# JasonQSY/Articulation3D

Hardware: AMD Instinct MI355X
Metric: frames/sec through PlaneRCNN detector at 480x640 (higher is better)
Workload: dtype f32 storage and accumulation; operands enter the matrix pipe with a 22-bit significand under ONE power-of-two block exponent per image (per ROI behind the poolers, per layer for filters): x*s = h + l in fp16, three fp16 MFMAs per k step (h.h + h.l + l.h). Elementwise law |y - y64| <= c (2^-22 sum|x|; 1 GPU; BASELINE configs[2]: full PlaneRCNN detector (ResNet50-FPN + RPN + ROIAlign + box/mask/plane/axis heads + depth head + NMS + mask paste + plane-offset LSQ + record pack), random-init weights with calibrated BN, synthetic 480x640 uint8 frames resident in HBM (arithmetic: see `dtype`)

## Files before the change

articulation3d_amd/csrc/conv_gemm.hip:

```cpp
#include "conv_common.h"
#include <stdarg.h>
#include <stdio.h>

static int conv_check(const a3d_conv_desc *d) {
    if (!d || (!d->x && !d->x_h2) || !d->w || (!d->y && !d->dot_y)) return A3D_ERR_ARG;
    if ((d->dot_w || d->dot_y) && d->phase != 5) return A3D_ERR_ARG;
    if (d->x_h2 && d->precision != 3) return A3D_ERR_ARG;
    if (d->B <= 0 || d->Ho <= 0 || d->Wo <= 0 || d->Cout <= 0) return A3D_ERR_ARG;
    if ((d->Cout & 3) || (d->Kpad & 31) || d->splitk < 1) return A3D_ERR_ARG;
    if (d->stem) {
        if (d->KH != 7 || d->KW != 7 || d->stride != 2 || d->pad != 3 || d->Kpad != 224 || d->Cin2 || d->ups) return A3D_ERR_ARG;
    } else {
        if ((d->Cin & 31) || (d->Cin2 & 31) || (d->Cin2 && !d->x2 && !d->x2_h2)) return A3D_ERR_ARG;
        if (d->Kpad < d->KH * d->KW * (d->Cin + d->Cin2)) return A3D_ERR_ARG;
    }
    if (d->pixshuf && (d->Cout & 15)) return A3D_ERR_ARG;
    if (d->phase < 0 || d->phase > 5 || (d->phase == 5 && d->precision != 3 && d->precision != 2)) return A3D_ERR_ARG;
    if (d->gate && (d->pixshuf || d->phase)) return A3D_ERR_ARG;
    if (d->io_bf16 && d->precision != 1) return A3D_ERR_ARG;
    if (d->splitk > 1 && !d->workspace) return A3D_ERR_ARG;
    if ((size_t)d->B * d->H * d->W >= ((size_t)1 << 31)) return A3D_ERR_UNSUPPORTED;
    return A3D_OK;
}

static thread_local char g_last_variant[160] = "";
void a3d_note_variant(const char *fmt, ...) {
    va_list ap;
    va_start(ap, fmt);
    vsnprintf(g_last_variant, sizeof(g_last_variant), fmt, ap);
    va_end(ap);
}
extern "C" const char *a3d_last_conv_variant(void) { return g_last_variant; }

extern "C" size_t a3d_conv_workspace_bytes(const a3d_conv_desc *d) {
    if (!d) return 0;
    if (d->tune == 0 && a3d_wino_fused_eligible(d)) return 0;
    if ((d->tune == 0 || d->tune == 7 || d->tune == 8 || (d->tune >= 23 && d->tune <= 25) || d->tune >= 200) && a3d_wino_eligible(d)) return a3d_wino_workspace_bytes(d);
    if (d->splitk <= 1) return 0;
    return (size_t)d->splitk * d->B * d->Ho * d->Wo * d->Cout * sizeof(float);
}

extern "C" int a3d_conv2d_nhwc_f32(const a3d_conv_desc *d, void *stream) {
    const int rc = conv_check(d);
    if (rc != A3D_OK) return rc;
    hipStream_t s = (hipStream_t)stream;
    a3d_begin();
    if (d->precision == 1) return a3d_conv_launch_bf16(d, s);
    if (d->precision == 2) {
        if ((d->tune == 0 || d->tune == 8 || d->tune == 24 || d->tune == 25) && d->workspace && d->w_wino && d->w_wino_x3 && ((d->Cin + d->Cin2) & 31) == 0 && a3d_wino_eligible(d)) return a3d_conv_launch_wino(d, s);
        return a3d_conv_launch_bf16x3(d, s);
    }
    if (d->precision == 3 && d->x_h2) return a3d_conv_launch_bf16x3_wide(d, s);
    if (d->precision == 3) {
        if ((d->tune == 0 || d->tune == 23 || d->tune == 24) && d->workspace && d->w_wino && d->w_wino_x3 && ((d->Cin + d->Cin2) & 31) == 0 && a3d_wino_eligible(d))
            return a3d_conv_launch_wino(d, s);
        return a3d_conv_launch_bf16x3(d, s);
    }
    if (d->precision != 0) return A3D_ERR_ARG;
    if (d->tune == 0 && a3d_wino_fused_eligible(d)) return a3d_conv_launch_wino_fused(d, s);
    if ((d->tune == 0 || d->tune == 7 || d->tune >= 200) && d->workspace && a3d_wino_eligible(d)) return a3d_conv_launch_wino(d, s);
    if (d->tune == 0 || d->tune == 6) {
        const int r1 = a3d_conv_launch_pw(d, s, d->tune == 6);
        if (r1 != A3D_ERR_UNSUPPORTED) return r1;
    }
    if (d->tune == 1) return A3D_ERR_UNSUPPORTED;
    return a3d_conv_launch_v2(d, s);
}

extern "C" int a3d_version(void) { return 1; }
```

articulation3d_amd/csrc/conv_wino.hip:

```cpp
#include "conv_common.h"
#include <stdlib.h>

typedef unsigned int u32x4 __attribute__((ext_vector_type(4)));

__global__ __launch_bounds__(256) void wino_input_kernel(const float *__restrict__ x, const float *__restrict__ x2,
                                                         float *__restrict__ V, int B, int H, int W, int Cin, int Cin2,
                                                         int ups, int Ty, int Tx) {
    const int C = Cin + Cin2, C4 = C >> 2;
    const int Hl = ups ? 2 * H : H, Wl = ups ? 2 * W : W;
    const size_t T = (size_t)B * Ty * Tx;
    const size_t total = T * C4;
    for (size_t i = (size_t)blockIdx.x * blockDim.x + threadIdx.x; i < total; i += (size_t)gridDim.x * blockDim.x) {
        const int c = (int)(i % C4) * 4;
        const size_t t = i / C4;
        const int tx = (int)(t % Tx);
        const size_t r = t / Tx;
        const int ty = (int)(r % Ty);
        const int b = (int)(r / Ty);
        const bool second = c >= Cin;
        const float *src = second ? x2 : x;
        const int cs = second ? Cin2 : Cin, cc = second ? c - Cin : c;
        f32x4 d[4][4];
#pragma unroll
        for (int p = 0; p < 4; ++p) {
            const int ly = 2 * ty - 1 + p;
#pragma unroll
            for (int q = 0; q < 4; ++q) {
                const int lx = 2 * tx - 1 + q;
                f32x4 v = {0.f, 0.f, 0.f, 0.f};
                if ((unsigned)ly < (unsigned)Hl && (unsigned)lx < (unsigned)Wl) {
                    const int sy = ups ? ly >> 1 : ly, sx = ups ? lx >> 1 : lx;
                    v = *reinterpret_cast<const f32x4 *>(src + (((size_t)b * H + sy) * W + sx) * cs + cc);
                }
                d[p][q] = v;
            }
        }
        f32x4 m[4][4];
#pragma unroll
        for (int q = 0; q < 4; ++q) {
            m[0][q] = d[0][q] - d[2][q];
            m[1][q] = d[1][q] + d[2][q];
            m[2][q] = d[2][q] - d[1][q];
            m[3][q] = d[1][q] - d[3][q];
        }
#pragma unroll
        for (int u = 0; u < 4; ++u) {
            const f32x4 v0 = m[u][0] - m[u][2], v1 = m[u][1] + m[u][2], v2 = m[u][2] - m[u][1], v3 = m[u][1] - m[u][3];
            float *o = V + ((size_t)(u * 4) * T + t) * C + c;
            *reinterpret_cast<f32x4 *>(o) = v0;
            *reinterpret_cast<f32x4 *>(o + T * C) = v1;
            *reinterpret_cast<f32x4 *>(o + 2 * T * C) = v2;
            *reinterpret_cast<f32x4 *>(o + 3 * T * C) = v3;
        }
    }
}

typedef unsigned int wi_u32x2 __attribute__((ext_vector_type(2)));
typedef unsigned int wi_u32x4 __attribute__((ext_vector_type(4)));
__global__ __launch_bounds__(256) void wino_input_h2_kernel(const float *__restrict__ x, const float *__restrict__ x2, unsigned char *__restrict__ Vs,
                                                            const float *__restrict__ in_amax, const float *__restrict__ in_amax2, int B, int H, int W,
                                                            int Cin, int Cin2, int ups, int Ty, int Tx, int t_off, int t_total) {
    const int C = Cin + Cin2;
    const int Hl = ups ? 2 * H : H, Wl = ups ? 2 * W : W;
    const size_t T = (size_t)B * Ty * Tx;
    const size_t tile = (size_t)t_total * 64;
    const int KC = C >> 5;
    const size_t witems = ((T + 7) / 8) * KC;
    const int lane = threadIdx.x & 63;
    for (size_t w = (size_t)blockIdx.x * (blockDim.x >> 6) + (threadIdx.x >> 6); w < witems; w += (size_t)gridDim.x * (blockDim.x >> 6)) {
        const int kcw = (int)(w % KC);
        const size_t t = (w / KC) * 8 + (lane >> 3);
        if (t >= T) continue;
        const int c = kcw * 32 + (lane & 7) * 4;
        const int tx = (int)(t % Tx);
        const size_t r = t / Tx;
        const int ty = (int)(r % Ty);
        const int b = (int)(r / Ty);
        const bool second = c >= Cin;
        const float *src = second ? x2 : x;
        const int cs = second ? Cin2 : Cin, cc = second ? c - Cin : c;
        float am = in_amax[b];
        if (in_amax2) am = fmaxf(am, in_amax2[b]);
        const float sv = 0.25f * a3d_pow2_scale(am);
        f32x4 d[4][4];
#pragma unroll
        for (int p = 0; p < 4; ++p) {
            const int ly = 2 * ty - 1 + p;
#pragma unroll
            for (int q = 0; q < 4; ++q) {
                const int lx = 2 * tx - 1 + q;
                f32x4 v = {0.f, 0.f, 0.f, 0.f};
                if ((unsigned)ly < (unsigned)Hl && (unsigned)lx < (unsigned)Wl) {
                    const int sy = ups ? ly >> 1 : ly, sx = ups ? lx >> 1 : lx;
                    v = *reinterpret_cast<const f32x4 *>(src + (((size_t)b * H + sy) * W + sx) * cs + cc);
                }
                d[p][q] = v;
            }
        }
        f32x4 m[4][4];
#pragma unroll
        for (int q = 0; q < 4; ++q) {
            m[0][q] = d[0][q] - d[2][q];
            m[1][q] = d[1][q] + d[2][q];
            m[2][q] = d[2][q] - d[1][q];
            m[3][q] = d[1][q] - d[3][q];
        }
        const int kc = c >> 5;
        unsigned char *oh = Vs + (size_t)kc * 2 * tile + ((size_t)t_off + t) * 64 + (c & 31) * 2;
        const size_t pstride = (size_t)KC * 2 * tile;
#pragma unroll
        for (int u = 0; u < 4; ++u) {
            const f32x4 vv[4] = {m[u][0] - m[u][2], m[u][1] + m[u][2], m[u][2] - m[u][1], m[u][1] - m[u][3]};
#pragma unroll
            for (int v = 0; v < 4; ++v) {
                h16x4 h, l;
                a3d_split2h(vv[v], sv, h, l);
                *reinterpret_cast<h16x4 *>(oh) = h;
                *reinterpret_cast<h16x4 *>(oh + tile) = l;
                oh += pstride;
            }
        }
    }
}

struct WinoArgs {
    const float *V;
    const float *U;
    const float *scale, *shift;
    const float *gate;
    float *y;
    int T, C, Cout, B, Hl, Wl, Ty, Tx, act;
    const __bf16 *U3;
    float *y_amax;
    const float *in_amax, *in_amax2;
    float w_scale;
    float *M;
    int abl;
    int Toff, Ttot;
    struct Levels {
        int n;
        int t0[6];
        int Ty[5], Tx[5], Hl[5], Wl[5];
        float *y[5];
        const float *in_amax[5];
        float *y_amax[5];
    } lv;
};
__device__ __forceinline__ void wino_level_of(const WinoArgs::Levels &L, const int t, int &l, int &tl) {
    l = 0;
#pragma unroll
    for (int k = 1; k < 5; ++k) l = (k < L.n && t >= L.t0[k]) ? k : l;
    int base = L.t0[0];
#pragma unroll
    for (int k = 1; k < 5; ++k) base = l == k ? L.t0[k] : base;
    tl = t - base;
}
template <typename V>
__device__ __forceinline__ V wino_level_sel(const V (&arr)[5], const int l) {
    V v = arr[0];
#pragma unroll
    for (int k = 1; k < 5; ++k) v = l == k ? arr[k] : v;
    return v;
}

__device__ __forceinline__ float wino_v_scale(const WinoArgs &a, const int b) {
    float m = a.in_amax[b];
    if (a.in_amax2) m = fmaxf(m, a.in_amax2[b]);
    return 0.25f * a3d_pow2_scale(m);
}

template <int TN, int BKT>
__global__ __launch_bounds__(256, TN == 1 ? 3 : 1) void wino_gemm_kernel(const WinoArgs a, const int ntiles, const int nblk) {
    constexpr int BM = 64, BN = 2 * TN * 32;
    constexpr int LK = BKT + 4, TPR = BKT / 4, RPP = 256 / TPR;
    constexpr int XR = (BM + RPP - 1) / RPP, WR = BN / RPP;
    constexpr int BUF = (BM + BN) * LK;
    static_assert(BN % RPP == 0 && (BM % RPP == 0 || BM < RPP), "loader pass must tile the operand rows");
    __shared__ __attribute__((aligned(16))) float lds[2 * BUF];
    __shared__ __attribute__((aligned(16))) float ss[2 * BN];

    const int tid = threadIdx.x, lane = tid & 63, wave = tid >> 6;
    const int wm = wave >> 1, wn = wave & 1;
    const int logical = a3d_xcd_remap(blockIdx.x, nblk);
    const int mt = logical / ntiles, nt = logical - mt * ntiles;
    const int t0 = mt * BM, n0 = nt * BN;
    const int lr = tid / TPR, lc = (tid % TPR) * 4;
    const size_t vplane = (size_t)a.T * a.C, uplane = (size_t)a.Cout * a.C;
    const unsigned vbytes = (unsigned)(vplane * 4), ubytes = (unsigned)(uplane * 4);
    const int KC = a.C / BKT;
    const int NIT = 16 * KC;

    int xoff[XR], woff[WR];
#pragma unroll
    for (int i = 0; i < XR; ++i) {
        const int rrow = lr + RPP * i;
        const int t = t0 + rrow;
        xoff[i] = (rrow < BM && t < a.T) ? (t * a.C + lc) * 4 : -1;
    }
#pragma unroll
    for (int i = 0; i < WR; ++i) {
        const int n = n0 + lr + RPP * i;
        woff[i] = n < a.Cout ? (n * a.C + lc) * 4 : -1;
    }
    f32x4 xsA[XR], wsA[WR], xsB[XR], wsB[WR];
// ... 1052 lines not shown
    *reinterpret_cast<bf16x4 *>(d + (size_t)rows * chunk) = m;
    *reinterpret_cast<bf16x4 *>(d + (size_t)rows * chunk * 2) = l;
}

extern "C" int a3d_split_bf16x3_chunk(const float *src, void *dst, int outer, int rows, int cols, int chunk, void *stream) {
    if (!src || !dst || outer <= 0 || rows <= 0 || cols <= 0 || (chunk != 16 && chunk != 32) || cols % chunk) return A3D_ERR_ARG;
    a3d_begin();
    const size_t total = (size_t)outer * rows * cols;
    hipLaunchKernelGGL(split_bf16x3_kernel, dim3((unsigned)((total / 4 + 255) / 256)), dim3(256), 0, (hipStream_t)stream, src, (__bf16 *)dst, rows, cols, chunk,
                       total);
    return a3d_check_launch();
}

__global__ __launch_bounds__(256) void split_f16x2_kernel(const float *__restrict__ src, _Float16 *__restrict__ dst, int rows, int cols, int chunk, float scale,
                                                          size_t total) {
    const size_t i = ((size_t)blockIdx.x * 256 + threadIdx.x) * 4;
    if (i >= total) return;
    const size_t per = (size_t)rows * cols;
    const size_t o = i / per, r = i - o * per;
    const int n = (int)(r / cols), c = (int)(r - (size_t)n * cols);
    h16x4 h, l;
    a3d_split2h(*reinterpret_cast<const f32x4 *>(src + i), scale, h, l);
    _Float16 *d = dst + o * 2 * per + ((size_t)(c / chunk) * 2 * rows + n) * chunk + (c % chunk);
    *reinterpret_cast<h16x4 *>(d) = h;
    *reinterpret_cast<h16x4 *>(d + (size_t)rows * chunk) = l;
}

extern "C" int a3d_split_f16x2_chunk(const float *src, void *dst, int outer, int rows, int cols, int chunk, float scale, void *stream) {
    if (!src || !dst || outer <= 0 || rows <= 0 || cols <= 0 || (chunk != 16 && chunk != 32) || cols % chunk || !(scale > 0.f)) return A3D_ERR_ARG;
    a3d_begin();
    const size_t total = (size_t)outer * rows * cols;
    hipLaunchKernelGGL(split_f16x2_kernel, dim3((unsigned)((total / 4 + 255) / 256)), dim3(256), 0, (hipStream_t)stream, src, (_Float16 *)dst, rows, cols, chunk,
                       scale, total);
    return a3d_check_launch();
}

extern "C" int a3d_split_bf16x3(const float *src, void *dst, int outer, int rows, int cols, void *stream) {
    return a3d_split_bf16x3_chunk(src, dst, outer, rows, cols, 32, stream);
}

int a3d_wino_eligible(const a3d_conv_desc *d) {
    if (!d->w_wino) return 0;
    if (d->KH != 3 || d->KW != 3 || d->stride != 1 || d->pad != 1) return 0;
    if (d->res || d->pixshuf || d->stem || d->splitk != 1 || d->m_dev) return 0;
    if (((d->Cin + d->Cin2) & 15) || (d->Cin & 3) || (d->Cin2 & 3) || (d->Cout & 3)) return 0;
    const int Hl = d->ups ? 2 * d->H : d->H, Wl = d->ups ? 2 * d->W : d->W;
    const size_t T = (size_t)d->B * ((Hl + 1) / 2) * ((Wl + 1) / 2);
    const size_t C = (size_t)d->Cin + d->Cin2;
    if (T * C * 4 >= ((size_t)1 << 32) || (size_t)d->Cout * C * 4 >= ((size_t)1 << 32)) return 0;
    return 1;
}

size_t a3d_wino_workspace_bytes(const a3d_conv_desc *d) {
    const int Hl = d->ups ? 2 * d->H : d->H, Wl = d->ups ? 2 * d->W : d->W;
    size_t T = (size_t)d->B * ((Hl + 1) / 2) * ((Wl + 1) / 2);
    if (d->precision == 3 && d->wino_t_total > 0) T = (size_t)d->wino_t_total;
    return 16 * T * ((size_t)d->Cin + d->Cin2) * sizeof(float);
}

extern "C" size_t a3d_wino_m_bytes(const a3d_conv_desc *d) {
    const long ps_max = a3d_dev_knob("A3D_WINO_PS_BLOCKS", 48);
    if (!d || d->precision != 3 || !a3d_wino_eligible(d)) return 0;
    const int C = d->Cin + d->Cin2;
    if ((C & 63) || ((d->Cout + 63) / 64) % 2 != 0) return 0;
    const int Hl = d->ups ? 2 * d->H : d->H, Wl = d->ups ? 2 * d->W : d->W;
    const size_t T = (size_t)d->B * ((Hl + 1) / 2) * ((Wl + 1) / 2);
    const long blocks4 = (long)((T + 127) / 128) * ((d->Cout + X3W_BN - 1) / X3W_BN);
    if (blocks4 > ps_max) return 0;
    return 16 * T * (size_t)d->Cout * sizeof(float);
}

static int wino_launch_input(const a3d_conv_desc *d, hipStream_t s) {
    const int Hl = d->ups ? 2 * d->H : d->H, Wl = d->ups ? 2 * d->W : d->W;
    const int Ty = (Hl + 1) / 2, Tx = (Wl + 1) / 2;
    const int C = d->Cin + d->Cin2;
    const size_t T = (size_t)d->B * Ty * Tx;
    const size_t total = T * (C / 4);
    size_t blocks = (total + 255) / 256;
    if (blocks > 16384) blocks = 16384;
    if (d->precision == 3) {
        if ((C & 31) || !d->in_amax) return A3D_ERR_ARG;
        if (d->wino_t_total && (d->wino_t_off < 0 || (size_t)d->wino_t_off + T > (size_t)d->wino_t_total)) return A3D_ERR_ARG;
        if ((size_t)(d->wino_t_total ? d->wino_t_total : T) * C * 4 >= ((size_t)1 << 32)) return A3D_ERR_UNSUPPORTED;
        hipLaunchKernelGGL(wino_input_h2_kernel, dim3((int)blocks), dim3(256), 0, s, d->x, d->x2, reinterpret_cast<unsigned char *>(d->workspace), d->in_amax,
                           d->in_amax2, d->B, d->H, d->W, d->Cin, d->Cin2, d->ups, Ty, Tx, d->wino_t_total ? d->wino_t_off : 0, d->wino_t_total ? d->wino_t_total : (int)T);
        return A3D_OK;
    }
    hipLaunchKernelGGL(wino_input_kernel, dim3((int)blocks), dim3(256), 0, s, d->x, d->x2, d->workspace, d->B, d->H, d->W,
                       d->Cin, d->Cin2, d->ups, Ty, Tx);
    return A3D_OK;
}

static int wino_launch_gemm(const a3d_conv_desc *d, hipStream_t s) {
    const int Hl = d->ups ? 2 * d->H : d->H, Wl = d->ups ? 2 * d->W : d->W;
    const int Ty = (Hl + 1) / 2, Tx = (Wl + 1) / 2;
    const size_t T = (size_t)d->B * Ty * Tx;
    WinoArgs a;
    a.V = d->workspace;
    a.U = d->w_wino;
    a.scale = d->scale;
    a.shift = d->shift;
    a.gate = d->gate;
    a.y = d->y;
    a.T = (int)T;
    a.C = d->Cin + d->Cin2;
    a.Cout = d->Cout;
    a.B = d->B;
    a.Hl = Hl;
    a.Wl = Wl;
    a.Ty = Ty;
    a.Tx = Tx;
    a.act = d->act;
    const int mtiles = (int)((T + 63) / 64);
    a.U3 = nullptr;
    a.y_amax = d->y_amax;
    a.in_amax = d->in_amax;
    a.in_amax2 = d->in_amax2;
    a.w_scale = d->w_scale;
    a.M = nullptr;
    a.abl = (int)a3d_dev_knob("A3D_WINO_ABL", 0);
    a.Toff = 0;
    a.Ttot = (int)T;
    a.lv.n = 1;
    for (int k = 0; k < 5; ++k) {
        a.lv.t0[k] = k == 0 ? 0 : (int)T;
        a.lv.Ty[k] = Ty;
        a.lv.Tx[k] = Tx;
        a.lv.Hl[k] = Hl;
        a.lv.Wl[k] = Wl;
        a.lv.y[k] = d->y;
        a.lv.in_amax[k] = d->in_amax;
        a.lv.y_amax[k] = d->y_amax;
    }
    a.lv.t0[5] = (int)T;
    if (d->wino_t_total) {
        if (d->precision != 3 || d->wino_t_off < 0 || (size_t)d->wino_t_off + T > (size_t)d->wino_t_total) return A3D_ERR_ARG;
        a.Toff = d->wino_t_off;
        a.Ttot = d->wino_t_total;
    }
    if (d->precision == 3) {
        if (!d->w_wino_x3 || (a.C & 31) || !d->in_amax || !(d->w_scale > 0.f) || ((d->Cout + 63) / 64) % 2 != 0 ||
            (size_t)16 * d->Cout * a.C * 4 >= ((size_t)1 << 32))
            return A3D_ERR_ARG;
        a.U3 = reinterpret_cast<const __bf16 *>(d->w_wino_x3);
        const int nt = (d->Cout + X3W_BN - 1) / X3W_BN;
        const int wmx = d->tune == 24 ? 2 : 4;
        static a3d_attr_once attr3;
        if (attr3.needed()) {
            if (hipFuncSetAttribute((const void *)wino_gemm_x3w_kernel<2, true>, hipFuncAttributeMaxDynamicSharedMemorySize, x3w_lds_bytes(2, 2)) != hipSuccess ||
                hipFuncSetAttribute((const void *)wino_gemm_x3w_kernel<4, true>, hipFuncAttributeMaxDynamicSharedMemorySize, x3w_lds_bytes(4, 2)) != hipSuccess ||
                hipFuncSetAttribute((const void *)wino_gemm_x3w_kernel<4, true, false, 1>, hipFuncAttributeMaxDynamicSharedMemorySize, x3w_lds_bytes(4, 2)) != hipSuccess ||
                hipFuncSetAttribute((const void *)wino_gemm_x3w_kernel<2, true, true>, hipFuncAttributeMaxDynamicSharedMemorySize, x3w_lds_bytes(2, 2)) != hipSuccess)
                return A3D_ERR_LAUNCH;
            attr3.mark();
        }
        if (d->wino_m && a3d_wino_m_bytes(d)) {
            a.M = d->wino_m;
            a3d_note_variant("wino_gemm_h2w_kernel<2> planes + wino_fold_kernel");
            hipLaunchKernelGGL((wino_gemm_x3w_kernel<2, true, true>), dim3(mtiles * nt, 16), dim3(256), x3w_lds_bytes(2, 2), s, a, nt, mtiles * nt);
            const size_t threads = T * (size_t)(d->Cout / 4);
            hipLaunchKernelGGL(wino_fold_kernel, dim3((unsigned)((threads + 255) / 256)), dim3(256), 0, s, a);
            return A3D_OK;
        }
        a3d_note_variant("wino_gemm_h2w_kernel<%d>", wmx);
        if (wmx == 4) {
            const int m4 = (int)((T + 127) / 128);
            if (d->tune == 23) hipLaunchKernelGGL((wino_gemm_x3w_kernel<4, true>), dim3(m4 * nt), dim3(512), x3w_lds_bytes(4, 2), s, a, nt, m4 * nt);
            else hipLaunchKernelGGL((wino_gemm_x3w_kernel<4, true, false, 1>), dim3(m4 * nt), dim3(512), x3w_lds_bytes(4, 2), s, a, nt, m4 * nt);
// ... 142 lines not shown
```

articulation3d_amd/ops.py:

```python
from __future__ import annotations

import ctypes as C
import math
import os
from dataclasses import dataclass
from typing import List, Optional, Sequence, Tuple

import torch

from . import _lib
from ._lib import ACT_LEAKY, ACT_NONE, ACT_RELU

GROUP_CAP = 1024
fptr_t = C.c_void_p

CONV_TIMING: Optional[list] = None

DEFAULT_PRECISION = int(os.environ.get("A3D_PRECISION", "3"))


def last_conv_variant() -> str:
    return _lib.lib().a3d_last_conv_variant().decode()


# ... 285 lines not shown
    publish()
    return t.data_ptr()


def _conv_desc(p: PackedConv, B: int, H: int, W: int, Cin: int, Cin2: int, Ho: int, Wo: int, act: Optional[int] = None,
               res_ups: bool = False) -> "_lib.ConvDesc":
    d = _lib.ConvDesc()
    d.w, d.scale, d.shift = _p(p.w), _p(p.scale), _p(p.shift)
    d.B, d.H, d.W, d.Cin, d.Cin2 = B, H, W, Cin, Cin2
    d.Ho, d.Wo, d.Cout = Ho, Wo, p.cols
    d.KH, d.KW, d.stride, d.pad = p.KH, p.KW, p.stride, p.pad
    d.Kpad, d.act = p.Kpad, p.act if act is None else act
    d.res_ups, d.pixshuf, d.stem, d.phase, d.splitk = int(res_ups), int(p.pixshuf), int(p.stem), int(p.phase), 1
    return d


def _y_amax(out: torch.Tensor) -> int:
    ya = getattr(out, "_a3d_amax", None)
    if ya is None or ya.numel() != out.shape[0]:
        ya = out._a3d_amax = amax_slot(out.shape[0], out.device)
    return ya.data_ptr()


def _image_blocks(B: int, nb: int, *ts):
    for s in range(0, B, nb):
        e = min(s + nb, B)
        yield s, e, [t if t is None or e - s == B else keep_amax(t[s:e], _amax_rows(t, s, e)) for t in ts]


CONV_TIMING_ONLY: Optional[frozenset] = None
_TIMED_VARIANTS: dict = {}
_ERR_UNSUPPORTED = -3


def _launch(fn, *args, precision: Optional[int] = None, rec=None, unsupported: bool = False) -> bool:
    global _LAST_PRECISION
    if precision is not None:
        _LAST_PRECISION = precision
    timed = CONV_TIMING is not None and rec is not None
    if timed:
        label, fl, shape, ex, pipe, key = rec()
        if CONV_TIMING_ONLY is not None:
            known = label if label is not None else _TIMED_VARIANTS.get(key)
            timed = known is None or known in CONV_TIMING_ONLY
        if timed:
            e0, e1 = (torch.cuda.Event(enable_timing=True) for _ in range(2))
            e0.record()
    rc = fn(*args, _stream())
    if rc:
        if unsupported and rc == _ERR_UNSUPPORTED:
            return False
        _lib.check(rc, fn.__name__)
    if timed:
        e1.record()
        if label is None:
            label = _TIMED_VARIANTS[key] = last_conv_variant()
        CONV_TIMING.append((label, fl, e0, e1, shape, ex, pipe, _stream()))
    return True


_WINO_SHARE: Optional[dict] = None
WINO_SHARE_ENABLED = os.environ.get("A3D_WINO_SHARE", "1") != "0"


class share_wino_input:

    def __init__(self, tensors: Sequence[torch.Tensor]):
        self.map = {t.data_ptr(): [t, None] for t in tensors} if WINO_SHARE_ENABLED else {}

    def __enter__(self):
        global _WINO_SHARE
        self.prev, _WINO_SHARE = _WINO_SHARE, self.map
        return self

    def __exit__(self, *exc):
        global _WINO_SHARE
        _WINO_SHARE = self.prev
        self.map = {}
        return False


_ADDR_LIMIT = (1 << 32) - 1
WINO_LEVELS = os.environ.get("A3D_WINO_LEVELS", "1") != "0"


def conv2d_levels(xs: Sequence[torch.Tensor], p: PackedConv) -> list:
    xs = list(xs)
    ok = (WINO_LEVELS and DEFAULT_PRECISION == 3 and AUDIT is None and 2 <= len(xs) <= 5 and p.w_wino is not None
          and p.pin_precision != 2 and p.KH == 3 and p.stride == 1 and p.pad == 1 and not (p.stem or p.phase or p.pixshuf)
          and all(x.is_cuda and x.dtype == torch.float32 and x.shape[0] == xs[0].shape[0] and x.shape[3] == p.Cin for x in xs)
          and p.Cin % 32 == 0 and p.Cin >= 256 and -(-p.cols // 64) % 2 == 0)
    if ok and _WINO_SHARE is not None:
        ok = all((_WINO_SHARE.get(x.data_ptr()) or [None, None])[1] is None for x in xs)
    tiles = [x.shape[0] * ((x.shape[1] + 1) // 2) * ((x.shape[2] + 1) // 2) for x in xs]
    total = sum(tiles)
    if not ok or total * p.Cin * 4 > _ADDR_LIMIT:
        return [conv2d(x, p) for x in xs]
    dev = xs[0].device
    w_h2, u_scale = weight_planes(p, "w_wino_h2"), filter_scale(p, wino=True)
    ws = torch.empty(16 * total * p.Cin, device=dev, dtype=torch.float32)
    descs = (_lib.ConvDesc * len(xs))()
    outs, off = [], 0
    shape = lambda: f"{xs[0].shape[0]}x[{'+'.join(str(x.shape[1]) + 'x' + str(x.shape[2]) for x in xs)}]x{p.Cin}->{p.cols} k3 s1"
    for k, x in enumerate(xs):
        _req(x)
        B, H, W, Cin = x.shape
        out = torch.empty((B, H, W, p.cols), device=dev, dtype=torch.float32)
        descs[k] = _conv_desc(p, B, H, W, Cin, 0, H, W)
        d = descs[k]
        d.x, d.y, d.precision = _p(x), _p(out), 3
        d.w_wino, d.w_wino_x3, d.w_scale = p.w_wino.data_ptr(), w_h2, u_scale
        d.in_amax = amax_of(x).data_ptr()
        d.y_amax = _y_amax(out)
        d.workspace = ws.data_ptr()
        d.wino_t_off, d.wino_t_total = off, total
        _launch(_lib.lib().a3d_wino_input_transform, C.byref(d), precision=3, rec=lambda: ("wino_input_kernel", 0.0, shape(), 0.0, "none", None))
        if _WINO_SHARE is not None:
            ent = _WINO_SHARE.get(x.data_ptr())
            if ent is not None and ent[0].shape == x.shape:
                ent[1:] = [ws, 3, (off, total)]
        off += tiles[k]
        outs.append(out)

    def rec():
        px = sum(x.shape[0] * x.shape[1] * x.shape[2] for x in xs)
        return "wino_gemm_h2w_kernel<4>", 2.0 * px * p.cols * 9 * p.Cin, shape(), 2.0 * total * 16 * p.cols * p.Cin, "f16x3", None

    _launch(_lib.lib().a3d_wino_gemm_levels, descs, len(xs), precision=3, rec=rec)
    return outs


def conv2d(x: torch.Tensor, p: PackedConv, *, x2: Optional[torch.Tensor] = None, res: Optional[torch.Tensor] = None,
           res_ups: bool = False, ups: bool = False, act: Optional[int] = None, splitk: int = 1,
           m_dev: Optional[torch.Tensor] = None, out: Optional[torch.Tensor] = None, tune: int = 0,
           wino: Optional[bool] = None, gate: Optional[torch.Tensor] = None, precision=None, out_dtype=None, dot=None) -> torch.Tensor:
    if AUDIT is not None and not AUDIT.busy and precision is None and x.dtype == torch.float32 and out_dtype is None and not p.phase:
        return AUDIT.conv2d(x, p, x2=x2, res=res, res_ups=res_ups, ups=ups, act=act, splitk=splitk, m_dev=m_dev, out=out, tune=tune, wino=wino, gate=gate)
    if x.dtype == torch.float16:
        if splitk != 1 or m_dev is not None or gate is not None or tune or out_dtype is not None or ups or dot is not None or wino or precision not in (None, 3):
            raise RuntimeError("pre-split (float16) activations run the dual-DMA fp16x2 kernel only: splitk, m_dev, gate, tune, out_dtype, ups, dot, "
                               "wino and any precision other than 3 are not available with them")
        return _conv2d_presplit(x, p, x2=x2, res=res, res_ups=res_ups, act=act, out=out)
    if out_dtype is not None or x.dtype == torch.bfloat16 or (res is not None and res.dtype == torch.bfloat16) or (gate is not None and gate.dtype == torch.bfloat16):
        return _conv2d_bf16_storage(x, p, res=res, res_ups=res_ups, act=act, out=out, gate=gate, precision=precision, out_dtype=out_dtype, tune=tune)
    _req(x)
    B = x.shape[0]
    if B > 1:
        Hl_, Wl_ = (2 * x.shape[1], 2 * x.shape[2]) if ups else (x.shape[1], x.shape[2])
        Ho_ = x.shape[1] if p.phase else (Hl_ + 2 * p.pad - p.KH) // p.stride + 1
        Wo_ = x.shape[2] if p.phase else (Wl_ + 2 * p.pad - p.KW) // p.stride + 1
        per_in = x.shape[1] * x.shape[2] * max(x.shape[3], 0 if x2 is None else x2.shape[3]) * 4
        per_out = Ho_ * Wo_ * p.cols * 4 * (4 if 0 < p.phase < 5 else 1) * max(1, int(splitk))
        if dot is not None:
            per_out = 9 * 4 * Ho_ * Wo_ * 4
        per_v = ((Hl_ + 1) // 2) * ((Wl_ + 1) // 2) * (x.shape[3] + (0 if x2 is None else x2.shape[3])) * 4 if p.w_wino is not None else 0
        per = max(per_in, per_out, per_v, 1)
        if B * per > _ADDR_LIMIT:
            if dot is not None:
                raise RuntimeError("tap-product epilogue (dot): the batch must fit one launch")
            return _conv2d_blocks(x, p, max(1, _ADDR_LIMIT // per), (Ho_, Wo_), x2=x2, res=res, res_ups=res_ups, ups=ups, act=act, splitk=splitk,
                                  m_dev=m_dev, out=out, tune=tune, wino=wino, gate=gate, precision=precision)
    return _conv2d_launch(x, p, x2=x2, res=res, res_ups=res_ups, ups=ups, act=act, splitk=splitk, m_dev=m_dev, out=out, tune=tune,
                          wino=wino, gate=gate, precision=precision, dot=dot)


def _conv2d_blocks(x, p, nb, hw_out, *, x2, res, out, gate, m_dev, **kw):
    B = x.shape[0]
    Ho, Wo = hw_out
    if out is None:
        shape = (B, 2 * Ho, 2 * Wo, p.cols // 4) if p.pixshuf else (B, Ho, Wo, p.cols)
        out = torch.empty(shape, device=x.device, dtype=torch.float32)
    recorded = []
    for s, e, (xb, x2b, rb, gb) in _image_blocks(B, nb, x, x2, res, gate):
        md = None if m_dev is None else (m_dev.reshape(1) - s).clamp(0, e - s).to(torch.int32)
        o = out[s:e]
        ya = getattr(out, "_a3d_amax", None)
        if ya is not None and ya.numel() == B:
            o._a3d_amax = ya[s:e]
        _conv2d_launch(xb, p, x2=x2b, res=rb, out=o, gate=gb, m_dev=md, **kw)
        recorded.append(getattr(o, "_a3d_amax", None))
    if getattr(out, "_a3d_amax", None) is None and all(r is not None for r in recorded):
        out._a3d_amax = torch.cat(recorded)
    return out


BF16_SPLITK = os.environ.get("A3D_BF16_SPLITK", "1") != "0"
BF16_SPLITK_AUTO = False
_BF16_SK_CFG = tuple(int(v) for v in os.environ.get("A3D_BF16_SPLITK_CFG", "128,256,12,24,8").split(","))


def _bf16_splitk(M: int, cols: int, Kpad: int) -> int:
    tiles = -(-M // 128) * -(-cols // 64)
    nk = Kpad // 32
    maxtiles, target, per, minnk, cap = _BF16_SK_CFG
    if not BF16_SPLITK or tiles > maxtiles or nk < minnk:
        return 1
    return int(max(1, min(cap, nk // per, target // tiles)))

# ... 48 lines not shown
    def rec():
        fl = 2.0 * B * Ho * Wo * p.cols * p.KH * p.KW * p.Cin
        return None, fl, f"{B}x{H}x{W}x{Cin}->{p.cols} k{p.KH} s{p.stride} io{int(d.io_bf16)}", fl, "bf16", key

    _launch(_lib.lib().a3d_conv2d_nhwc_f32, C.byref(d), precision=1, rec=rec)
    return out


def presplit_f16x2(x: torch.Tensor, x2: Optional[torch.Tensor] = None):
    _req(x)
    B, n = x.shape[0], x.numel() // x.shape[0]
    ax, ax2 = amax_of(x), (None if x2 is None else amax_of(_req(x2)))
    outs = []
    for t in ((x,) if x2 is None else (x, x2)):
        nt = t.numel() // B
        o = torch.empty(tuple(t.shape[:-1]) + (t.shape[-1] // 16, 2, 16), device=t.device, dtype=torch.float16)
        _lib.check(_lib.lib().a3d_presplit_f16x2(t.data_ptr(), o.data_ptr(), ax.data_ptr(), _p(ax2), B, nt, _stream()), "a3d_presplit_f16x2")
        o._a3d_amax = ax if x2 is None else torch.maximum(ax, ax2)
        outs.append(o)
    return outs[0] if x2 is None else tuple(outs)


def _conv2d_presplit(x, p: PackedConv, *, x2=None, res=None, res_ups=False, act=None, out=None) -> torch.Tensor:
    if DEFAULT_PRECISION != 3:
        raise RuntimeError("pre-split activations belong to the fp16x2 arithmetic (A3D_PRECISION=3)")
    ok = lambda t: t.is_cuda and t.is_contiguous() and t.dtype == torch.float16 and t.dim() == 6 and t.shape[4:] == (2, 16)
    if not ok(x) or (x2 is not None and not ok(x2)):
        raise RuntimeError("expected contiguous pre-split fp16 tensors [B, H, W, C/16, 2, 16]")
    B, H, W = x.shape[:3]
    Cin = x.shape[3] * 16
    Cin2 = 0 if x2 is None else x2.shape[3] * 16
    assert Cin + Cin2 == p.Cin and not (p.stem or p.pixshuf or p.phase) and p.presplit and p.Kpad == p.KH * p.KW * p.Cin, "plain direct layers only"
    Ho = (H + 2 * p.pad - p.KH) // p.stride + 1
    Wo = (W + 2 * p.pad - p.KW) // p.stride + 1
    if out is None:
        out = torch.empty((B, Ho, Wo, p.cols), device=x.device, dtype=torch.float32)
    per_image = max(H * W * max(Cin, Cin2), Ho * Wo * p.cols) * 4
    if B * per_image > _ADDR_LIMIT:
        ya = out._a3d_amax = amax_slot(B, x.device)
        for s, e, (xb, x2b, rb) in _image_blocks(B, max(1, _ADDR_LIMIT // per_image), x, x2, res):
            o = out[s:e]
            o._a3d_amax = ya[s:e]
            _conv2d_presplit(xb, p, x2=x2b, res=rb, res_ups=res_ups, act=act, out=o)
        return out
    a = getattr(x, "_a3d_amax", None)
    if a is None or a.numel() != B:
        raise RuntimeError("a pre-split tensor carries the per-image maxima it was scaled by (_a3d_amax)")
    d = _conv_desc(p, B, H, W, Cin, Cin2, Ho, Wo, act=act, res_ups=res_ups)
    d.x_h2, d.x2_h2, d.res, d.y = x.data_ptr(), _p(x2), _p(res), out.data_ptr()
    d.precision = 3
    d.tune = int(os.environ.get("A3D_XD_TUNE", "0"))
    d.in_amax = a.data_ptr()
    d.w_scale, d.w_x3 = filter_scale(p), weight_planes(p, "w_h2")
    d.y_amax = _y_amax(out)

    def rec():
        fl = 2.0 * B * Ho * Wo * p.cols * p.KH * p.KW * p.Cin
        return None, fl, f"{B}x{H}x{W}x{Cin + Cin2}->{p.cols} k{p.KH} s{p.stride} presplit", fl, "f16x3", (id(p), B, H, W, Cin, Cin2, "presplit")

    _launch(_lib.lib().a3d_conv2d_nhwc_f32, C.byref(d), precision=3, rec=rec)
    return out


class _amax_rows:

    def __init__(self, t, s, e):
        a = getattr(t, "_a3d_amax", None)
        self._a3d_amax = None if a is None or a.numel() != t.shape[0] else a[s:e]
        self.shape = (e - s,)


def _check_res(res: torch.Tensor, B: int, Ho: int, Wo: int, cols: int, res_ups: bool) -> None:
    _req(res)
    want = (B, Ho >> 1, Wo >> 1, cols) if res_ups else (B, Ho, Wo, cols)
    if tuple(res.shape) != want or (res_ups and (Ho % 2 or Wo % 2)):
        raise ValueError(f"residual of shape {tuple(res.shape)} for an output grid [{B}, {Ho}, {Wo}, {cols}]{' (res_ups)' if res_ups else ''}: expected {want}")


_PIPE = {0: "f32", 1: "bf16", 2: "bf16x6", 3: "f16x3"}


def _arithmetic(p: PackedConv, default: int, wino_tune: int, precision, Cin: int, Cin2: int, *, ups: bool, splitk: int, tune: int, wino,
                x2: bool, res: bool, gate: bool, m_dev: bool) -> Tuple[int, bool, int]:
    wino_ok = (p.w_wino is not None and not res and splitk == 1 and not m_dev and (tune in (0, 7, 8, 23, 24, 25) or tune >= 200) and not ups
               and (wino if wino is not None else True))
    if precision is None or precision == "bf16x3":
        mode = default if precision is None else 2
        if mode == 3 and p.pin_precision == 2:
            mode = 2
        plain = not (p.stem or ups or p.phase or p.pixshuf or x2 or splitk != 1 or m_dev) and p.Kpad == p.KH * p.KW * p.Cin
        if mode == 1:
            precision = 1 if plain and p.Cin % 32 == 0 else 0
        elif mode in (2, 3):
            x3_ok = p.stem and not ups and splitk == 1 and not m_dev and not x2 and not res
            x3_ok = x3_ok or (not (p.stem or ups or m_dev) and p.Kpad == p.KH * p.KW * p.Cin
                     and not (p.pixshuf and (res or gate))
                     and (splitk == 1 or (p.presplit and p.Kpad >= 4096 and p.cols >= 192 and -(-p.cols // 256) * 256 <= p.cols + p.cols // 4
                                          and not p.phase and not gate and not p.pixshuf))
                     and (not x2 or Cin2 == Cin) and Cin % 16 == 0 and not (p.phase and res))
            precision = 2 if tune == 0 and ((x3_ok and not wino_ok) or (wino_ok and (Cin + Cin2) % 32 == 0)) else 0
            if precision == 2 and mode == 3:
                precision = 3
        else:
            precision = 0
    use_wino = wino_ok and (precision == 0 or (precision in (2, 3) and tune in (0, 8, 23, 24, 25) and (Cin + Cin2) % 32 == 0))
    if use_wino and precision == 3 and (-(-p.cols // 64) % 2 or (Cin + Cin2 < 256 and wino is None)):
        use_wino = False
    if use_wino and precision == 3 and tune == 0 and wino_tune:
        tune = wino_tune
    return int(precision), use_wino, int(tune)


def _conv2d_launch(x: torch.Tensor, p: PackedConv, *, x2: Optional[torch.Tensor] = None, res: Optional[torch.Tensor] = None,
                   res_ups: bool = False, ups: bool = False, act: Optional[int] = None, splitk: int = 1,
                   m_dev: Optional[torch.Tensor] = None, out: Optional[torch.Tensor] = None, tune: int = 0,
                   wino: Optional[bool] = None, gate: Optional[torch.Tensor] = None, precision=None, dot=None) -> torch.Tensor:
    _req(x)
    plan_key = None
    if (LAUNCH_PLANS and CONV_TIMING is None and x2 is None and m_dev is None and out is None and gate is None and dot is None and not ups and splitk == 1
            and tune == 0 and wino is None and precision is None and act is None and not (p.phase or p.pixshuf or p.stem) and p.presplit
            and (_WINO_SHARE is None or x.data_ptr() not in _WINO_SHARE)):
        plan_key = (DEFAULT_PRECISION, WINO_TUNE, p.pin_precision, x.shape, None if res is None else tuple(res.shape), bool(res_ups),
                    WINO_PLANE_SPLIT, BF16_SPLITK_AUTO, BF16_SPLITK, x.device, p.w.data_ptr())
        plans = p.__dict__.get("_plans")
        plan = plans.get(plan_key) if plans else None
        if plan is not None:
            proto, oshape, need_in, need_y, ws_n, m_n, prec = plan
            out = torch.empty(oshape, device=x.device, dtype=torch.float32)
            d = _lib.ConvDesc.from_buffer_copy(proto)
            d.x, d.y = x.data_ptr(), out.data_ptr()
            if res is not None:
                _check_res(res, oshape[0], d.Ho, d.Wo, d.Cout, res_ups)
                d.res = res.data_ptr()
            if need_in:
                d.in_amax = amax_of(x).data_ptr()
            if need_y:
                ya = out._a3d_amax = amax_slot(oshape[0], x.device)
                d.y_amax = ya.data_ptr()
            if ws_n:
                ws = torch.empty(ws_n, device=x.device, dtype=torch.float32)
                d.workspace = ws.data_ptr()
            if m_n:
                wino_m = torch.empty(m_n, device=x.device, dtype=torch.float32)
                d.wino_m = wino_m.data_ptr()
            _launch(_lib.lib().a3d_conv2d_nhwc_f32, C.byref(d), precision=prec)
            return out
    B, H, W, Cin = x.shape
    Cin2 = 0
    if x2 is not None:
        _req(x2)
        Cin2 = x2.shape[3]
        assert x2.shape[:3] == x.shape[:3]
    if not p.stem:
        assert Cin + Cin2 == p.Cin, (Cin, Cin2, p.Cin)
    Hl, Wl = (2 * H, 2 * W) if ups else (H, W)
    Ho = (Hl + 2 * p.pad - p.KH) // p.stride + 1
    Wo = (Wl + 2 * p.pad - p.KW) // p.stride + 1
    if p.phase:
        assert not ups and out is not None, "phase convs run on the source grid and fill a shared [B,2H,2W,C] output"
        Ho, Wo = H, W
        if p.phase == 5:
            assert precision in (2, 3) and (dot is not None or tuple(out.shape) == (B, 2 * H, 2 * W, p.cols // 4)), "the fused four-phase form belongs to the split-operand arithmetics"
    if res is not None:
        _check_res(res, B, Ho, Wo, p.cols, res_ups)
    if out is None:
        shape = (B, 2 * Ho, 2 * Wo, p.cols // 4) if p.pixshuf else (B, Ho, Wo, p.cols)
        out = torch.empty(shape, device=x.device, dtype=torch.float32)
    d = _conv_desc(p, B, H, W, Cin, Cin2, Ho, Wo, act=act, res_ups=res_ups)
    d.x, d.x2, d.res, d.y = _p(x), _p(x2), _p(res), _p(out)
    d.ups, d.splitk, d.m_dev = int(ups), int(splitk), _p(m_dev)
    if gate is not None:
        assert tuple(_req(gate).shape) == tuple(out.shape), (gate.shape, out.shape)
        d.gate = gate.data_ptr()
    if dot is not None:
        assert p.phase == 5 and precision == 3
        d.dot_w, d.dot_y = _req(dot[0]).data_ptr(), _req(dot[1]).data_ptr()
        d.y = None
    precision, use_wino, tune = _arithmetic(p, DEFAULT_PRECISION, WINO_TUNE, precision, Cin, Cin2, ups=ups, splitk=splitk, tune=tune, wino=wino,
                                            x2=x2 is not None, res=res is not None, gate=gate is not None, m_dev=m_dev is not None)
    d.precision, d.tune = precision, tune
    if precision == 1 and p.w_b16 is not None:
        d.w_bf16 = p.w_b16.data_ptr()
    if (precision == 1 and splitk == 1 and BF16_SPLITK_AUTO and not (p.stem or ups or p.phase or p.pixshuf or x2 is not None or m_dev is not None or res_ups)
            and p.Kpad == p.KH * p.KW * p.Cin and p.Cin % 32 == 0):
        splitk = _bf16_splitk(B * Ho * Wo, p.cols, p.Kpad)
        d.splitk = splitk
    if precision == 3:
        d.in_amax = amax_of(x).data_ptr()
        if x2 is not None:
            d.in_amax2 = amax_of(x2).data_ptr()
        d.w_scale = filter_scale(p)
    if precision in (2, 3) and (DEFAULT_PRECISION == 3 or precision == 3) and not p.pixshuf:
        d.y_amax = _y_amax(out)
    if use_wino:
        d.w_wino = p.w_wino.data_ptr()
        if p.w_wino_cm is not None and precision == 0 and tune == 0:
            d.w_wino_cm = p.w_wino_cm.data_ptr()
        if precision == 3:
            d.w_scale = filter_scale(p, wino=True)
            d.w_wino_x3 = weight_planes(p, "w_wino_h2")
        elif precision == 2:
            d.w_wino_x3 = weight_planes(p, "w_wino_x3")
    elif precision == 3 and p.presplit and p.Kpad % 16 == 0:
        d.w_x3 = weight_planes(p, "w_h2")
    elif (precision == 2 and p.presplit and p.cols >= 192 and p.Kpad % 16 == 0 and (p.Kpad >= 4096 or tune == 9 or p.phase == 5)
            and not (p.stem or p.pixshuf)):
        d.w_x3 = weight_planes(p, "w_x3")
    ws = None
    fused_wino = False
    shared = None
    nbytes = mbytes = 0
    if use_wino or splitk > 1:
        if use_wino and _WINO_SHARE is not None and x2 is None:
            shared = _WINO_SHARE.get(x.data_ptr())
            if shared is not None and (shared[0].shape != x.shape or tune not in (0, 23, 24)):
                shared = None
            if shared is not None and shared[1] is not None and len(shared) > 2 and shared[2] != precision:
                shared = None
        if shared is not None:
            d.w_wino_cm = None
            if len(shared) > 3 and shared[1] is not None:
                d.wino_t_off, d.wino_t_total = shared[3]
        nbytes = _lib.lib().a3d_conv_workspace_bytes(C.byref(d))
        fused_wino = use_wino and nbytes == 0
        if shared is not None and shared[1] is not None:
            ws = shared[1]
            assert ws.numel() * 4 == nbytes
            d.workspace = ws.data_ptr()
        elif nbytes:
            ws = torch.empty(nbytes // 4, device=x.device, dtype=torch.float32)
            d.workspace = ws.data_ptr()
        if use_wino and precision == 3 and WINO_PLANE_SPLIT:
            mbytes = _lib.lib().a3d_wino_m_bytes(C.byref(d))
            if mbytes:
                wino_m = torch.empty(mbytes // 4, device=x.device, dtype=torch.float32)
                d.wino_m = wino_m.data_ptr()
    have_v = False
    if shared is not None:
        have_v, shared[1] = shared[1] is not None, ws
        if len(shared) > 2:
            shared[2] = precision
        else:
            shared.append(precision)

    def rec(label=None):
        k_real = 147 if p.stem else p.KH * p.KW * p.Cin
        shape = f"{B}x{H}x{W}x{Cin + Cin2}->{p.cols} k{p.KH} s{p.stride}{' ups' if ups else ''}{' sk%d' % splitk if splitk > 1 else ''}"
        if label is not None:
            return label, 0.0, shape, 0.0, "none", None
        fl = 2.0 * B * Ho * Wo * p.cols * (9 * p.Cin if p.phase else k_real)
        if use_wino:
            ex = 2.0 * B * ((Ho + 1) // 2) * ((Wo + 1) // 2) * 16 * p.cols * p.Cin
        else:
            ex = 2.0 * B * Ho * Wo * p.cols * (4 * p.Cin if p.phase == 5 else k_real)
        return None, fl, shape, ex, _PIPE[precision], (id(p), B, H, W, bool(ups), int(splitk), precision, tune, res is not None, x2 is not None, shared is not None)

    L = _lib.lib()
    if use_wino and not fused_wino and (shared is not None or CONV_TIMING is not None):
        if not have_v:
            _launch(L.a3d_wino_input_transform, C.byref(d), precision=precision, rec=lambda: rec("wino_input_kernel"))
        _launch(L.a3d_wino_gemm, C.byref(d), precision=precision, rec=rec)
        return out
    _launch(L.a3d_conv2d_nhwc_f32, C.byref(d), precision=precision, rec=rec)
    if plan_key is not None:
        if p.__dict__.get("_plans") is None or len(p._plans) > 64:
            p._plans = {}
        p._plans[plan_key] = (bytes(d), tuple(out.shape), bool(d.in_amax), bool(d.y_amax), nbytes // 4 if ws is not None else 0,
                              mbytes // 4 if d.wino_m else 0, precision)
    return out


LAUNCH_PLANS = os.environ.get("A3D_LAUNCH_PLANS", "1") != "0"
B2B_FUSED = os.environ.get("A3D_B2B", "1") != "0"
B2B_MIN_PIXELS = 128 * 512
B2B_PAIRS = ((64, 64),)


def conv2d_b2b(x: torch.Tensor, p1: PackedConv, res: torch.Tensor, p2: PackedConv):
    if not B2B_FUSED or DEFAULT_PRECISION != 3 or AUDIT is not None or not x.is_cuda or x.dtype != torch.float32:
        return None
    B, H, W, Cin = x.shape
    M = B * H * W
    if (p1.KH, p1.KW, p1.stride, p1.pad, p2.KH, p2.KW, p2.stride, p2.pad) != (1, 1, 1, 0, 1, 1, 1, 0) or p1.pin_precision == 2:
        return None
    if (Cin, p2.cols) not in B2B_PAIRS or p1.Cin != Cin or p2.Cin != p1.cols or p1.cols % 64 or not (p1.presplit and p2.presplit):
        return None
    if p1.Kpad != Cin or p2.Kpad != p2.Cin or p1.pixshuf or p2.pixshuf or p1.phase or p2.phase or p1.stem or p2.stem:
        return None
    if M < B2B_MIN_PIXELS or M * p1.cols * 4 >= (1 << 31) or res is None or tuple(res.shape) != (B, H, W, p1.cols):
        return None
    _req(x)
    _req(res)
    y = torch.empty((B, H, W, p1.cols), device=x.device, dtype=torch.float32)
    z = torch.empty((B, H, W, p2.cols), device=x.device, dtype=torch.float32)
    d1, d2 = _conv_desc(p1, B, H, W, Cin, 0, H, W), _conv_desc(p2, B, H, W, p2.Cin, 0, H, W)
    d1.x, d1.res, d1.y, d1.y_amax = x.data_ptr(), res.data_ptr(), y.data_ptr(), _y_amax(y)
    d2.x, d2.y, d2.y_amax = y.data_ptr(), z.data_ptr(), _y_amax(z)
    d1.precision, d2.precision = 3, 2
# ... 514 lines not shown
```

Measured before the change: 1568 frames/s.

## Add row-walking Winograd input transform that reuses overlapping tile rows

Adds a new Winograd F(2,3) input-transform kernel for the split-fp16 path. Each wavefront owns one 32-channel chunk and eight tile columns and walks a vertical segment of tile rows, carrying the two overlapping input rows forward so each input row is loaded about once instead of twice. Loads go through buffer resources with the per-image scale hoisted, and the split h/l planes are written with nontemporal stores. The old grid-stride kernel is kept as a fallback, selectable through tune 26 or an environment variable, and is used when Tx is not a multiple of eight or there are too few walkers. The cost is less parallelism per launch and more complex indexing and dispatch.

After: 1580 frames/s, median of 6. No clear change (+0.8%).

```diff
diff --git a/articulation3d_amd/csrc/conv_gemm.hip b/articulation3d_amd/csrc/conv_gemm.hip
--- a/articulation3d_amd/csrc/conv_gemm.hip
+++ b/articulation3d_amd/csrc/conv_gemm.hip
@@ -35,7 +35,7 @@
 extern "C" size_t a3d_conv_workspace_bytes(const a3d_conv_desc *d) {
     if (!d) return 0;
     if (d->tune == 0 && a3d_wino_fused_eligible(d)) return 0;
-    if ((d->tune == 0 || d->tune == 7 || d->tune == 8 || (d->tune >= 23 && d->tune <= 25) || d->tune >= 200) && a3d_wino_eligible(d)) return a3d_wino_workspace_bytes(d);
+    if ((d->tune == 0 || d->tune == 7 || d->tune == 8 || (d->tune >= 23 && d->tune <= 27) || d->tune >= 200) && a3d_wino_eligible(d)) return a3d_wino_workspace_bytes(d);
     if (d->splitk <= 1) return 0;
     return (size_t)d->splitk * d->B * d->Ho * d->Wo * d->Cout * sizeof(float);
 }
@@ -52,7 +52,7 @@
     }
     if (d->precision == 3 && d->x_h2) return a3d_conv_launch_bf16x3_wide(d, s);
     if (d->precision == 3) {
-        if ((d->tune == 0 || d->tune == 23 || d->tune == 24) && d->workspace && d->w_wino && d->w_wino_x3 && ((d->Cin + d->Cin2) & 31) == 0 && a3d_wino_eligible(d))
+        if ((d->tune == 0 || d->tune == 23 || d->tune == 24 || d->tune == 26 || d->tune == 27) && d->workspace && d->w_wino && d->w_wino_x3 && ((d->Cin + d->Cin2) & 31) == 0 && a3d_wino_eligible(d))
             return a3d_conv_launch_wino(d, s);
         return a3d_conv_launch_bf16x3(d, s);
     }
diff --git a/articulation3d_amd/csrc/conv_wino.hip b/articulation3d_amd/csrc/conv_wino.hip
--- a/articulation3d_amd/csrc/conv_wino.hip
+++ b/articulation3d_amd/csrc/conv_wino.hip
@@ -57,9 +57,9 @@
 
 typedef unsigned int wi_u32x2 __attribute__((ext_vector_type(2)));
 typedef unsigned int wi_u32x4 __attribute__((ext_vector_type(4)));
-__global__ __launch_bounds__(256) void wino_input_h2_kernel(const float *__restrict__ x, const float *__restrict__ x2, unsigned char *__restrict__ Vs,
-                                                            const float *__restrict__ in_amax, const float *__restrict__ in_amax2, int B, int H, int W,
-                                                            int Cin, int Cin2, int ups, int Ty, int Tx, int t_off, int t_total) {
+__global__ __launch_bounds__(256) void wino_input_h2_flat_kernel(const float *__restrict__ x, const float *__restrict__ x2, unsigned char *__restrict__ Vs,
+                                                                 const float *__restrict__ in_amax, const float *__restrict__ in_amax2, int B, int H, int W,
+                                                                 int Cin, int Cin2, int ups, int Ty, int Tx, int t_off, int t_total) {
     const int C = Cin + Cin2;
     const int Hl = ups ? 2 * H : H, Wl = ups ? 2 * W : W;
     const size_t T = (size_t)B * Ty * Tx;
@@ -120,6 +120,75 @@
                 oh += pstride;
             }
         }
+    }
+}
+
+__global__ __launch_bounds__(256) void wino_input_h2_kernel(const float *__restrict__ x, const float *__restrict__ x2, unsigned char *__restrict__ Vs,
+                                                            const float *__restrict__ in_amax, const float *__restrict__ in_amax2, int B, int H, int W,
+                                                            int Cin, int Cin2, int ups, int Ty, int Tx, int t_off, int t_total, int seg, int nseg) {
+    const int C = Cin + Cin2, KC = C >> 5;
+    const int Hl = ups ? 2 * H : H, Wl = ups ? 2 * W : W;
+    const size_t tile = (size_t)t_total * 64;
+    const int lane = threadIdx.x & 63, wpw = blockDim.x >> 6, ng = Tx >> 3;
+    unsigned bid = blockIdx.x;
+    const int kcw = (int)(bid % (KC / wpw)) * wpw + __builtin_amdgcn_readfirstlane(threadIdx.x >> 6);
+    bid /= KC / wpw;
+    const int tx = (int)(bid % ng) * 8 + (lane >> 3);
+    bid /= ng;
+    const int sg = (int)(bid % nseg), b = (int)(bid / nseg);
+    const int ty0 = sg * seg, ty1 = min(Ty, ty0 + seg);
+    if (b >= B || ty0 >= ty1) return;
+    const bool second = kcw * 32 >= Cin;
+    const int cs = second ? Cin2 : Cin, c0 = second ? kcw * 32 - Cin : kcw * 32;
+    const float *img = (second ? x2 : x) + (size_t)b * H * W * cs + c0;
+    const __amdgpu_buffer_rsrc_t rs = a3d_rsrc_uniform(img, (unsigned)(((size_t)H * W * cs - c0) * 4));
+    float am = in_amax[b];
+    if (in_amax2) am = fmaxf(am, in_amax2[b]);
+    const float sv = 0.25f * a3d_pow2_scale(am);
+    int xo[4];
+#pragma unroll
+    for (int q = 0; q < 4; ++q) {
+        const int lx = 2 * tx - 1 + q;
+        xo[q] = (unsigned)lx < (unsigned)Wl ? ((ups ? lx >> 1 : lx) * cs + (lane & 7) * 4) * 4 : -1;
+    }
+    auto load_row = [&](const int ly, f32x4(&row)[4]) {
+        const bool in = (unsigned)ly < (unsigned)Hl;
+        const int soff = min(max(ups ? ly >> 1 : ly, 0), H - 1) * W * cs * 4;
+#pragma unroll
+        for (int q = 0; q < 4; ++q) row[q] = a3d_load4(rs, in ? xo[q] : -1, soff);
+    };
+    f32x4 d[4][4];
+#pragma unroll
+    for (int p = 0; p < 2; ++p) load_row(2 * ty0 - 1 + p, d[p]);
+    unsigned char *const run0 = Vs + (size_t)kcw * 2 * tile;
+    unsigned voff = (unsigned)(((size_t)t_off + ((size_t)b * Ty + ty0) * Tx + tx) * 64 + (lane & 7) * 8);
+    const size_t pstride = (size_t)KC * 2 * tile;
+#pragma unroll 1
+    for (int ty = ty0; ty < ty1; ++ty) {
+        load_row(2 * ty + 1, d[2]);
+        load_row(2 * ty + 2, d[3]);
+        unsigned char *run = run0;
+#pragma unroll
+        for (int u = 0; u < 4; ++u) {
+            f32x4 m[4];
+#pragma unroll
+            for (int q = 0; q < 4; ++q) m[q] = u == 0 ? d[0][q] - d[2][q] : (u == 1 ? d[1][q] + d[2][q] : (u == 2 ? d[2][q] - d[1][q] : d[1][q] - d[3][q]));
+            const f32x4 vv[4] = {m[0] - m[2], m[1] + m[2], m[2] - m[1], m[1] - m[3]};
+#pragma unroll
+            for (int v = 0; v < 4; ++v) {
+                h16x4 h, l;
+                a3d_split2h(vv[v], sv, h, l);
+                __builtin_nontemporal_store(h, reinterpret_cast<h16x4 *>(run + voff));
+                __builtin_nontemporal_store(l, reinterpret_cast<h16x4 *>(run + tile + voff));
+                run += pstride;
+            }
+        }
+#pragma unroll
+        for (int q = 0; q < 4; ++q) {
+            d[0][q] = d[2][q];
+            d[1][q] = d[3][q];
+        }
+        voff += (unsigned)Tx * 64;
     }
 }
 
@@ -1338,8 +1407,22 @@
         if ((C & 31) || !d->in_amax) return A3D_ERR_ARG;
         if (d->wino_t_total && (d->wino_t_off < 0 || (size_t)d->wino_t_off + T > (size_t)d->wino_t_total)) return A3D_ERR_ARG;
         if ((size_t)(d->wino_t_total ? d->wino_t_total : T) * C * 4 >= ((size_t)1 << 32)) return A3D_ERR_UNSUPPORTED;
-        hipLaunchKernelGGL(wino_input_h2_kernel, dim3((int)blocks), dim3(256), 0, s, d->x, d->x2, reinterpret_cast<unsigned char *>(d->workspace), d->in_amax,
-                           d->in_amax2, d->B, d->H, d->W, d->Cin, d->Cin2, d->ups, Ty, Tx, d->wino_t_total ? d->wino_t_off : 0, d->wino_t_total ? d->wino_t_total : (int)T);
+        const int t_off = d->wino_t_total ? d->wino_t_off : 0, t_total = d->wino_t_total ? d->wino_t_total : (int)T;
+        const int ng = Tx >> 3, KC = C >> 5;
+        if (d->tune != 26 && (Tx & 7) == 0 && (size_t)d->H * d->W * (d->Cin > d->Cin2 ? d->Cin : d->Cin2) * 4 < ((size_t)1 << 31)) {
+            const int nseg = (Ty + 15) / 16, seg = (Ty + nseg - 1) / nseg;
+            const int wpw = KC % 4 == 0 ? 4 : (KC % 2 == 0 ? 2 : 1);
+            const size_t walkers = (size_t)d->B * nseg * ng * KC;
+            if ((walkers >= 640 || d->tune == 27) && walkers / wpw < ((size_t)1 << 31)) {
+                a3d_note_variant("wino_input_h2_kernel seg %d x %d", seg, nseg);
+                hipLaunchKernelGGL(wino_input_h2_kernel, dim3((unsigned)(walkers / wpw)), dim3(64 * wpw), 0, s, d->x, d->x2, reinterpret_cast<unsigned char *>(d->workspace),
+                                   d->in_amax, d->in_amax2, d->B, d->H, d->W, d->Cin, d->Cin2, d->ups, Ty, Tx, t_off, t_total, seg, nseg);
+                return A3D_OK;
+            }
+        }
+        a3d_note_variant("wino_input_h2_flat_kernel");
+        hipLaunchKernelGGL(wino_input_h2_flat_kernel, dim3((int)blocks), dim3(256), 0, s, d->x, d->x2, reinterpret_cast<unsigned char *>(d->workspace), d->in_amax,
+                           d->in_amax2, d->B, d->H, d->W, d->Cin, d->Cin2, d->ups, Ty, Tx, t_off, t_total);
         return A3D_OK;
     }
     hipLaunchKernelGGL(wino_input_kernel, dim3((int)blocks), dim3(256), 0, s, d->x, d->x2, d->workspace, d->B, d->H, d->W,
diff --git a/articulation3d_amd/ops.py b/articulation3d_amd/ops.py
--- a/articulation3d_amd/ops.py
+++ b/articulation3d_amd/ops.py
@@ -391,6 +391,7 @@
 
 _ADDR_LIMIT = (1 << 32) - 1
 WINO_LEVELS = os.environ.get("A3D_WINO_LEVELS", "1") != "0"
+WINO_INPUT_WALK = os.environ.get("A3D_WINO_INPUT_WALK", "1") != "0"
 
 
 def conv2d_levels(xs: Sequence[torch.Tensor], p: PackedConv) -> list:
@@ -423,6 +424,7 @@
         d.y_amax = _y_amax(out)
         d.workspace = ws.data_ptr()
         d.wino_t_off, d.wino_t_total = off, total
+        d.tune = 0 if WINO_INPUT_WALK else 26
         _launch(_lib.lib().a3d_wino_input_transform, C.byref(d), precision=3, rec=lambda: ("wino_input_kernel", 0.0, shape(), 0.0, "none", None))
         if _WINO_SHARE is not None:
             ent = _WINO_SHARE.get(x.data_ptr())
@@ -637,7 +639,7 @@
 
 def _arithmetic(p: PackedConv, default: int, wino_tune: int, precision, Cin: int, Cin2: int, *, ups: bool, splitk: int, tune: int, wino,
                 x2: bool, res: bool, gate: bool, m_dev: bool) -> Tuple[int, bool, int]:
-    wino_ok = (p.w_wino is not None and not res and splitk == 1 and not m_dev and (tune in (0, 7, 8, 23, 24, 25) or tune >= 200) and not ups
+    wino_ok = (p.w_wino is not None and not res and splitk == 1 and not m_dev and (tune in (0, 7, 8, 23, 24, 25, 26, 27) or tune >= 200) and not ups
                and (wino if wino is not None else True))
     if precision is None or precision == "bf16x3":
         mode = default if precision is None else 2
@@ -658,7 +660,7 @@
                 precision = 3
         else:
             precision = 0
-    use_wino = wino_ok and (precision == 0 or (precision in (2, 3) and tune in (0, 8, 23, 24, 25) and (Cin + Cin2) % 32 == 0))
+    use_wino = wino_ok and (precision == 0 or (precision in (2, 3) and (tune in (0, 8, 23, 24, 25) or (precision == 3 and tune in (26, 27))) and (Cin + Cin2) % 32 == 0))
     if use_wino and precision == 3 and (-(-p.cols // 64) % 2 or (Cin + Cin2 < 256 and wino is None)):
         use_wino = False
     if use_wino and precision == 3 and tune == 0 and wino_tune:
@@ -676,7 +678,7 @@
             and tune == 0 and wino is None and precision is None and act is None and not (p.phase or p.pixshuf or p.stem) and p.presplit
             and (_WINO_SHARE is None or x.data_ptr() not in _WINO_SHARE)):
         plan_key = (DEFAULT_PRECISION, WINO_TUNE, p.pin_precision, x.shape, None if res is None else tuple(res.shape), bool(res_ups),
-                    WINO_PLANE_SPLIT, BF16_SPLITK_AUTO, BF16_SPLITK, x.device, p.w.data_ptr())
+                    WINO_PLANE_SPLIT, WINO_INPUT_WALK, BF16_SPLITK_AUTO, BF16_SPLITK, x.device, p.w.data_ptr())
         plans = p.__dict__.get("_plans")
         plan = plans.get(plan_key) if plans else None
         if plan is not None:
@@ -733,6 +735,8 @@
         d.y = None
     precision, use_wino, tune = _arithmetic(p, DEFAULT_PRECISION, WINO_TUNE, precision, Cin, Cin2, ups=ups, splitk=splitk, tune=tune, wino=wino,
                                             x2=x2 is not None, res=res is not None, gate=gate is not None, m_dev=m_dev is not None)
+    if use_wino and precision == 3 and tune == 0 and not WINO_INPUT_WALK:
+        tune = 26
     d.precision, d.tune = precision, tune
     if precision == 1 and p.w_b16 is not None:
         d.w_bf16 = p.w_b16.data_ptr()
@@ -768,7 +772,7 @@
     if use_wino or splitk > 1:
         if use_wino and _WINO_SHARE is not None and x2 is None:
             shared = _WINO_SHARE.get(x.data_ptr())
-            if shared is not None and (shared[0].shape != x.shape or tune not in (0, 23, 24)):
+            if shared is not None and (shared[0].shape != x.shape or tune not in (0, 23, 24, 26, 27)):
                 shared = None
             if shared is not None and shared[1] is not None and len(shared) > 2 and shared[2] != precision:
                 shared = None
```
